# edenartlab/sd-lora-trainer

Measured on AMD Instinct MI355X. Metric: training images/sec, SDXL 1024px rank-16 LoRA, 1/2/4/8 GPU (job-parallel), higher is better.
Workload: dtype bf16

## Files before the change

### sd-lora-trainer_amd/csrc/attn.hip

```cpp
#include <cstdlib>
#include "common.h"
#include "../../include/sdlt_kernels.h"
#include "attn32.h"

namespace {

#ifdef SDLT_ATTN_TRACE
#define TR() do { if (tr) trb[trn++] = clock64(); } while (0)
#else
#define TR() do {} while (0)
#endif

constexpr float LOG2E = 1.4426950408889634f;

__device__ __forceinline__ bf16x8 pack8(const float* a, const float* b) {
  union { uint4 u; bf16x8 v; } c;
  c.u.x = pack2bf(a[0], a[1]); c.u.y = pack2bf(a[2], a[3]);
  c.u.z = pack2bf(b[0], b[1]); c.u.w = pack2bf(b[2], b[3]);
  return c.v;
}
__device__ __forceinline__ bf16x8 ld_frag_global(const bf16_t* p, bool ok) {
  union { uint4 u; bf16x8 v; } c;
  c.u = ok ? *(const uint4*)p : make_uint4(0, 0, 0, 0);
  return c.v;
// ... 1033 lines not shown
    return s;
  }();
  return sw;
}

struct AttnPlan {
  int route = 0;
  int dp = 64, ks = 1;
  bool dv48 = false, five = false, prep = false, splitsum = false;
  dim3 grid, grid2;
  int block = 256, smem = 0, smem2 = 0;
  int nq_roles = 0;
};
int attn32_ks(int env, bool two) { return env >= 4 ? 4 : env >= 2 ? 2 : env > 0 ? 1 : two ? 2 : 1; }

int attn_plan_fwd(const sdlt_attn_params& p, const AttnSwitches& sw, AttnPlan& pl) {
  int rc = attn_check(p, "sdlt_attn_fwd");
  if (rc) return rc;
  if (p.ldo % 4) SDLT_FAIL(SDLT_ERR_ALIGN, "sdlt_attn_fwd: ldo %% 4");
  pl = AttnPlan{};
  pl.dp = attn_dp(p.d);
  pl.grid = dim3((p.Nq + 63) / 64, p.H, p.B);
  if (sw.r32 && sdlt_attn32_ok(p) && ((uintptr_t)p.O % 16) == 0 && (p.ldo % 8) == 0) {
    pl.route = SDLT_ATTN_ROUTE_FWD32;
    pl.ks = attn32_ks(sw.ks32_fwd, p.Nk >= 128);
    pl.block = 128 * pl.ks;
    pl.smem = sdlt_attn32_fwd(pl.ks).smem;
    return SDLT_OK;
  }
  const bool ks2 = pl.dp == 64 && sw.ks == 2 && p.Nk >= 256 && (int64_t)pl.grid.x * pl.grid.y * pl.grid.z <= 512;
  pl.route = ks2 ? SDLT_ATTN_ROUTE_FWD16_KS2 : SDLT_ATTN_ROUTE_FWD16;
  pl.ks = ks2 ? 2 : 1;
  pl.dv48 = !ks2 && sw.dv48 && pl.dp == 64 && p.d <= 48;
  pl.block = 256 * pl.ks;
  pl.smem = smem_fwd(pl.dp, pl.ks);
  return SDLT_OK;
}

int attn_plan_bwd(const sdlt_attn_params& p, const AttnSwitches& sw, AttnPlan& pl) {
  int rc = attn_check_bwd(p, "sdlt_attn_bwd", false);
  if (rc) return rc;
  if (p.qsplit < 1) SDLT_FAIL(SDLT_ERR_SHAPE, "sdlt_attn_bwd: qsplit=%d", p.qsplit);
  if (!p.dK || !p.dV || (p.lddk % 4) || (p.lddv % 4) || (p.qsplit > 1 && (!p.dK32 || !p.dV32 || (p.ld32 % 4))))
    SDLT_FAIL(SDLT_ERR_SHAPE, "sdlt_attn_bwd: dK/dV outputs for qsplit=%d", p.qsplit);
  pl = AttnPlan{};
  pl.dp = attn_dp(p.d);
  const int tq = (p.Nq + 63) / 64, tk = (p.Nk + 63) / 64;
  if (p.qsplit > 1 && !p.causal && p.Nk <= 128 && p.Nkp <= 128 && pl.dp <= 96) {
    const bool roles = sw.roles && pl.dp == 64;
    pl.route = roles ? SDLT_ATTN_ROUTE_BWD_CROSS_ROLES : SDLT_ATTN_ROUTE_BWD_CROSS;
    pl.five = sw.five && p.Nk > 64 && p.Nk <= 80;
    if (roles) pl.nq_roles = p.qsplit / sw.qdiv > 0 ? p.qsplit / sw.qdiv : 1;
    pl.grid = dim3(pl.nq_roles + p.qsplit, p.H, p.B);
    pl.smem = roles ? smem_cross_roles(pl.dp) : smem_cross(pl.dp);
    pl.splitsum = !p.defer_splitsum;
    return SDLT_OK;
  }
  if (p.qsplit == 1 && !p.accumulate_dq && !p.accumulate_dk && (int64_t)(tq + tk) * p.H * p.B <= 2048) {
    const int64_t groups = (int64_t)p.B * p.Nqp * p.H;
    if (groups >= (1 << 22)) SDLT_FAIL(SDLT_ERR_UNSUPPORTED, "sdlt_attn_bwd: B * Nq * H = %lld rows (the D pre-pass indexes < 2^22)", (long long)groups);
    pl.prep = !p.d_ready;
    pl.grid = dim3(tq + tk, p.H, p.B);
    if (sw.r32 && sdlt_attn32_ok(p) && ((uintptr_t)p.L % 16) == 0 && ((uintptr_t)p.D % 16) == 0 &&
        (((uintptr_t)p.dQ | (uintptr_t)p.dK | (uintptr_t)p.dV) % 16) == 0 && ((p.lddq | p.lddk | p.lddv) % 8) == 0) {
      pl.route = SDLT_ATTN_ROUTE_BWD_BOTH32;
      pl.ks = attn32_ks(sw.ks32_bwd, p.Nk >= 128 && p.Nq >= 128);
      pl.block = 128 * pl.ks;
      pl.smem = sdlt_attn32_bwd_both(pl.ks).smem;
    } else {
      pl.route = SDLT_ATTN_ROUTE_BWD_BOTH16;
      pl.smem = smem_both(pl.dp);
    }
    return SDLT_OK;
  }
  if (p.accumulate_dq || p.accumulate_dk) SDLT_FAIL(SDLT_ERR_UNSUPPORTED, "sdlt_attn_bwd: accumulate_dq/dk exist for the single-pass cross-attention kernel only");
  if (p.qsplit > 1 && (((uintptr_t)p.dK32 | (uintptr_t)p.dV32) & 15 || (p.ld32 & 3) || ((p.H * p.d) & 3)))
    SDLT_FAIL(SDLT_ERR_ALIGN, "sdlt_attn_bwd: the dK / dV slabs of a query-split backward need 16-byte rows (ld32 %% 4, C %% 4)");
  pl.route = SDLT_ATTN_ROUTE_BWD_SPLIT;
  pl.dv48 = sw.dv48 && pl.dp == 64 && p.d <= 48;
  pl.grid = dim3(tq, p.H, p.B);
  pl.grid2 = dim3(tk * p.qsplit, p.H, p.B);
  pl.smem = smem_fwd(pl.dp);
  pl.smem2 = smem_both(pl.dp);
  pl.splitsum = p.qsplit > 1;
  return SDLT_OK;
}

// ... 135 lines not shown
```

### sd-lora-trainer_amd/csrc/attn32.h

```cpp
#pragma once
#include <hip/hip_runtime.h>
#include "../../include/sdlt_kernels.h"
bool sdlt_attn32_ok(const sdlt_attn_params& p);
struct sdlt_attn32_kernel { void (*fn)(const sdlt_attn_params); int smem; };
sdlt_attn32_kernel sdlt_attn32_fwd(int ks);
sdlt_attn32_kernel sdlt_attn32_bwd_both(int ks);
```

### sd-lora-trainer_amd/csrc/attn32.hip

```cpp
#include "common.h"
#include "../../include/sdlt_kernels.h"
#include "attn32.h"

namespace {

constexpr float LOG2E = 1.4426950408889634f;
typedef float f32x16 __attribute__((ext_vector_type(16)));
constexpr int TILE = 64 * 128;

__device__ __forceinline__ int sw32(int row) { return (((row >> 1) & 1) << 2) | ((row >> 2) & 3); }
__device__ __forceinline__ int rmap(int rho) { return (rho & 0x13) | ((rho & 4) << 1) | ((rho & 8) >> 1); }

struct WgId { int x, y, z; };
__device__ __forceinline__ WgId xcd_wg() {
  const int gx = gridDim.x, gy = gridDim.y, n = gx * gy * gridDim.z;
  const int L = blockIdx.x + gx * (blockIdx.y + gy * blockIdx.z);
  const int k = L & 7, slot = L >> 3, q = n >> 3, r = n & 7;
  const int logical = (k < r ? k * (q + 1) : r * (q + 1) + (k - r) * q) + slot;
  WgId w;
  const int t = div_small_u(logical, gx);
  w.x = logical - t * gx;
  w.z = gridDim.z == 1 ? 0 : div_small_u(t, gy);
  w.y = t - w.z * gy;
  return w;
}

__device__ __forceinline__ void tile_dma(const bf16_t* src, int64_t ld, char* dst, int w2, int lane) {
#pragma unroll
  for (int pc = 0; pc < 4; ++pc) {
    const int piece = w2 * 4 + pc;
    const int r = piece * 8 + (lane >> 3);
    glds16(src + (int64_t)r * ld + (((lane & 7) ^ sw32(r)) << 3), dst + piece * 1024);
  }
}

template <int OFF>
__device__ __forceinline__ bf16x8 lds_b128(uint32_t a) {
  bf16x8 v;
  asm volatile("ds_read_b128 %0, %1 offset:%2" : "=v"(v) : "v"(a), "n"(OFF));
  return v;
}
template <int OFF>
__device__ __forceinline__ bf16x4 lds_tr(uint32_t a) {
  bf16x4 v;
  asm volatile("ds_read_b64_tr_b16 %0, %1 offset:%2" : "=v"(v) : "v"(a), "n"(OFF));
  return v;
}
template <int N>
__device__ __forceinline__ void wait_lgkm() { asm volatile("s_waitcnt lgkmcnt(%0)" ::"n"(N) : "memory"); }
__device__ __forceinline__ void pin(bf16x8& v) { asm volatile("" : "+v"(v)); }
__device__ __forceinline__ void pin(bf16x4& v) { asm volatile("" : "+v"(v)); }
template <int BLK>
__device__ __forceinline__ void rows_issue(bf16x8 (&f)[4], uint32_t tile, const int (&row)[4]) {
#pragma unroll
  for (int kk = 0; kk < 4; ++kk) f[kk] = lds_b128<BLK * 4096>(tile + row[kk]);
}
__device__ __forceinline__ void rows_pin(bf16x8 (&f)[4]) {
#pragma unroll
  for (int kk = 0; kk < 4; ++kk) pin(f[kk]);
}
struct TrFrag { bf16x4 v[4]; };
template <int CH>
__device__ __forceinline__ void tr_issue(TrFrag& f, uint32_t tile, const int (&t1)[2], const int (&t2)[2]) {
  f.v[0] = lds_tr<CH * 2048>(tile + t1[0]);
  f.v[1] = lds_tr<CH * 2048>(tile + t2[0]);
  f.v[2] = lds_tr<CH * 2048>(tile + t1[1]);
  f.v[3] = lds_tr<CH * 2048>(tile + t2[1]);
}
__device__ __forceinline__ void tr_pin(TrFrag& f) {
#pragma unroll
  for (int k = 0; k < 4; ++k) pin(f.v[k]);
}
__device__ __forceinline__ bf16x8 tr_get(const TrFrag& f, int db) { return __builtin_shufflevector(f.v[2 * db], f.v[2 * db + 1], 0, 1, 2, 3, 4, 5, 6, 7); }
__device__ __forceinline__ uint32_t lds_addr(const char* p) { return (uint32_t)(uintptr_t)(__attribute__((address_space(3))) const char*)p; }
__device__ __forceinline__ bf16x8 ld8(const bf16_t* p) {
  union { uint4 u; bf16x8 v; } c;
  c.u = *(const uint4*)p;
  return c.v;
}
__device__ __forceinline__ bf16x8 pack8v(const f32x16& v, int c2) {
  union { uint4 u; bf16x8 b; } c;
  c.u.x = pack2bf(v[8 * c2 + 0], v[8 * c2 + 1]); c.u.y = pack2bf(v[8 * c2 + 2], v[8 * c2 + 3]);
  c.u.z = pack2bf(v[8 * c2 + 4], v[8 * c2 + 5]); c.u.w = pack2bf(v[8 * c2 + 6], v[8 * c2 + 7]);
  return c.b;
}
__device__ __forceinline__ float half_max(float v) {
  auto r = __builtin_amdgcn_permlane32_swap(__float_as_uint(v), __float_as_uint(v), false, false);
  return fmaxf(__uint_as_float(r[0]), __uint_as_float(r[1]));
}
__device__ __forceinline__ float half_sum(float v) {
  auto r = __builtin_amdgcn_permlane32_swap(__float_as_uint(v), __float_as_uint(v), false, false);
  return __uint_as_float(r[0]) + __uint_as_float(r[1]);
}
#ifndef SDLT_A32_STORE16
#define SDLT_A32_STORE16 1
#endif
__device__ __forceinline__ void store_pair(bf16_t* p, int hl, uint2 ev, uint2 od) {
#if SDLT_A32_STORE16
  auto x = __builtin_amdgcn_permlane32_swap(ev.x, od.x, false, false);
  auto y = __builtin_amdgcn_permlane32_swap(ev.y, od.y, false, false);
  *(uint4*)p = make_uint4(x[0], y[0], x[1], y[1]);
#else
  *(uint2*)(p - 4 * hl) = ev;
  *(uint2*)(p - 4 * hl + 8) = od;
#endif
}

__device__ __forceinline__ void wait_dma_barrier() {
  asm volatile("s_waitcnt vmcnt(0)" ::: "memory");
  __syncthreads();
}

struct FragOff {
  int row[4];
  int t1[2], t2[2];
};
__device__ __forceinline__ FragOff frag_offsets(int lane) {
  FragOff f;
  const int hl = lane >> 5, c = lane & 31, rr = rmap(c);
#pragma unroll
  for (int kk = 0; kk < 4; ++kk) f.row[kk] = rr * 128 + (((2 * kk + hl) ^ sw32(rr)) << 4);
  const int g = lane >> 4, i = lane & 15;
  const int R = 8 * (g >> 1) + (i >> 2), swl = (((i >> 3) & 1) << 2) | ((g >> 1) << 1), chl = 2 * (g & 1) + ((i & 3) >> 1);
#pragma unroll
  for (int db = 0; db < 2; ++db) {
    f.t1[db] = R * 128 + (((4 * db + chl) ^ swl) << 4) + (i & 1) * 8;
    f.t2[db] = (R + 4) * 128 + (((4 * db + chl) ^ swl ^ 1) << 4) + (i & 1) * 8;
  }
  return f;
}

#define MFMA32(a, b, c) __builtin_amdgcn_mfma_f32_32x32x16_bf16(a, b, c, 0, 0, 0)

#ifndef SDLT_A32_DMA_SPLIT
#define SDLT_A32_DMA_SPLIT 1
#endif

#ifdef SDLT_ATTN32_TRACE
#define TR32_DECL(BUF_, ON_) long long* tr_ = (long long*)(BUF_); int tn_ = 0; const bool tron_ = (ON_) && tr_ != nullptr
#define TR32() do { if (tron_ && tn_ < 500) { __builtin_amdgcn_sched_barrier(0); tr_[tn_++] = clock64(); __builtin_amdgcn_sched_barrier(0); } } while (0)
#else
#define TR32_DECL(BUF_, ON_)
#define TR32() do { } while (0)
#endif

template <int KS>
__global__ __launch_bounds__(128 * KS) void attn32_fwd_kernel(const sdlt_attn_params p) {
  extern __shared__ __attribute__((aligned(16))) char smem[];
  const WgId wg = xcd_wg();
  const int b = wg.z, h = wg.y, q0 = wg.x * 64;
  const int lane = threadIdx.x & 63, wv = __builtin_amdgcn_readfirstlane(threadIdx.x >> 6);
  const int grp = wv >> 1, w2 = wv & 1, hl = lane >> 5, c = lane & 31;
  const int hc = h * 64;
  const int q = q0 + w2 * 32 + c;
  const bf16_t* Kb = (const bf16_t*)p.K + (int64_t)b * p.Nkp * p.ldk + hc;
  const bf16_t* Vb = (const bf16_t*)p.V + (int64_t)b * p.Nkp * p.ldv + hc;
  char* ring = smem + grp * (4 * TILE);
  const int ntile = p.Nk >> 6, niter = (ntile + KS - 1) / KS;
  if (grp < ntile) {
    tile_dma(Kb + (int64_t)grp * 64 * p.ldk, p.ldk, ring, w2, lane);
    tile_dma(Vb + (int64_t)grp * 64 * p.ldv, p.ldv, ring + TILE, w2, lane);
  }
  bf16x8 qf[4];
  {
    const bf16_t* qp = (const bf16_t*)p.Q + ((int64_t)b * p.Nqp + q) * p.ldq + hc + 8 * hl;
#pragma unroll
    for (int kk = 0; kk < 4; ++kk) qf[kk] = ld8(qp + 16 * kk);
  }
  const FragOff fo = frag_offsets(lane);
  float m = -1e30f, lsum = 0.f;
  f32x16 o[2];
#pragma unroll
  for (int db = 0; db < 2; ++db)
#pragma unroll
    for (int r = 0; r < 16; ++r) o[db][r] = 0.f;
  const float sl2 = p.scale * LOG2E;
  TR32_DECL(p.D, wg.x == 0 && wg.y == 0 && wg.z == 0 && threadIdx.x == 0);
  TR32();
  wait_dma_barrier();
  for (int it = 0; it < niter; ++it) {
    TR32();
    const int t = it * KS + grp;
    const char* Ks = ring + (it & 1) * (2 * TILE);
    const char* Vs = Ks + TILE;
    char* nb = ring + ((it + 1) & 1) * (2 * TILE);
    const bool more = t + KS < ntile;
#if SDLT_A32_DMA_SPLIT == 0
    if (more) {
      tile_dma(Kb + (int64_t)(t + KS) * 64 * p.ldk, p.ldk, nb, w2, lane);
      tile_dma(Vb + (int64_t)(t + KS) * 64 * p.ldv, p.ldv, nb + TILE, w2, lane);
    }
#endif
    TR32();
    if (t < ntile) {
      const uint32_t ka = lds_addr(Ks), va = lds_addr(Vs);
      bf16x8 k0f[4], k1f[4];
      TrFrag vt[4];
      rows_issue<0>(k0f, ka, fo.row);
      rows_issue<1>(k1f, ka, fo.row);
      tr_issue<0>(vt[0], va, fo.t1, fo.t2);
      tr_issue<1>(vt[1], va, fo.t1, fo.t2);
      f32x16 s[2];
#pragma unroll
      for (int blk = 0; blk < 2; ++blk)
#pragma unroll
        for (int r = 0; r < 16; ++r) s[blk][r] = 0.f;
      wait_lgkm<12>();
      rows_pin(k0f);
#pragma unroll
      for (int kk = 0; kk < 4; ++kk) s[0] = MFMA32(k0f[kk], qf[kk], s[0]);
#if SDLT_A32_DMA_SPLIT
      if (more) tile_dma(Kb + (int64_t)(t + KS) * 64 * p.ldk, p.ldk, nb, w2, lane);
#endif
      tr_issue<2>(vt[2], va, fo.t1, fo.t2);
      tr_issue<3>(vt[3], va, fo.t1, fo.t2);
      wait_lgkm<15>();
      rows_pin(k1f);
#pragma unroll
      for (int kk = 0; kk < 4; ++kk) s[1] = MFMA32(k1f[kk], qf[kk], s[1]);
#if SDLT_A32_DMA_SPLIT
      if (more) tile_dma(Vb + (int64_t)(t + KS) * 64 * p.ldv, p.ldv, nb + TILE, w2, lane);
#endif
      __builtin_amdgcn_sched_barrier(0);
      TR32();
      float tmax = s[0][0];
#pragma unroll
      for (int blk = 0; blk < 2; ++blk)
#pragma unroll
        for (int r = 0; r < 16; ++r) tmax = fmaxf(tmax, s[blk][r]);
      tmax = half_max(tmax);
      const float mn = fmaxf(m, tmax * sl2);
      const float alpha = __builtin_amdgcn_exp2f(m - mn);
      m = mn;
      float rs = 0.f;
#pragma unroll
      for (int blk = 0; blk < 2; ++blk)
#pragma unroll
        for (int r = 0; r < 16; ++r) {
          const float pv = __builtin_amdgcn_exp2f(__builtin_fmaf(s[blk][r], sl2, -mn));
          s[blk][r] = pv;
          rs += pv;
        }
      lsum = lsum * alpha + rs;
#pragma unroll
      for (int db = 0; db < 2; ++db)
#pragma unroll
        for (int r = 0; r < 16; ++r) o[db][r] *= alpha;
      __builtin_amdgcn_sched_barrier(0);
      TR32();
      wait_lgkm<0>();
#pragma unroll
      for (int ch = 0; ch < 4; ++ch) tr_pin(vt[ch]);
#pragma unroll
      for (int ch = 0; ch < 4; ++ch) {
        const bf16x8 pf = pack8v(s[ch >> 1], ch & 1);
#pragma unroll
        for (int db = 0; db < 2; ++db) o[db] = MFMA32(tr_get(vt[ch], db), pf, o[db]);
      }
    }
    TR32();
    wait_dma_barrier();
  }
  TR32();
  lsum = half_sum(lsum);
  if constexpr (KS > 1) {
    float* mg = (float*)smem + (((grp - 1) * 2 + w2) * 64 + lane) * 36;
    if (grp > 0) {
      mg[0] = m;
      mg[1] = lsum;
#pragma unroll
      for (int db = 0; db < 2; ++db)
#pragma unroll
        for (int j = 0; j < 4; ++j) *(f32x4*)(mg + 4 + db * 16 + j * 4) = (f32x4){o[db][4 * j], o[db][4 * j + 1], o[db][4 * j + 2], o[db][4 * j + 3]};
    }
    __syncthreads();
    if (grp > 0) return;
#pragma unroll
    for (int g2 = 1; g2 < KS; ++g2) {
      const float* sg = (const float*)smem + (((g2 - 1) * 2 + w2) * 64 + lane) * 36;
      const float m1 = sg[0], l1 = sg[1];
      const float mn = fmaxf(m, m1), a0 = __builtin_amdgcn_exp2f(m - mn), a1 = __builtin_amdgcn_exp2f(m1 - mn);
      m = mn;
      lsum = lsum * a0 + l1 * a1;
#pragma unroll
// ... 14 lines not shown
  bf16_t* op = (bf16_t*)p.O + ((int64_t)b * p.Nqp + q) * p.ldo + hc + 8 * hl;
#pragma unroll
  for (int db = 0; db < 2; ++db)
#pragma unroll
    for (int jp = 0; jp < 2; ++jp) {
      uint2 w[2];
#pragma unroll
      for (int e = 0; e < 2; ++e) {
        const int j = 2 * jp + e;
        w[e].x = pack2bf(o[db][4 * j] * inv, o[db][4 * j + 1] * inv);
        w[e].y = pack2bf(o[db][4 * j + 2] * inv, o[db][4 * j + 3] * inv);
      }
      store_pair(op + 32 * db + 16 * jp, hl, w[0], w[1]);
    }
}

template <int KS>
__device__ __forceinline__ void attn32_dq_body(const sdlt_attn_params& p, char* smem, const int bx, const WgId wg) {
  const int b = wg.z, h = wg.y, q0 = bx * 64;
  const int lane = threadIdx.x & 63, wv = __builtin_amdgcn_readfirstlane(threadIdx.x >> 6);
  const int grp = wv >> 1, w2 = wv & 1, hl = lane >> 5, c = lane & 31;
  const int hc = h * 64;
  const int q = q0 + w2 * 32 + c;
  const bf16_t* Kb = (const bf16_t*)p.K + (int64_t)b * p.Nkp * p.ldk + hc;
  const bf16_t* Vb = (const bf16_t*)p.V + (int64_t)b * p.Nkp * p.ldv + hc;
  char* ring = smem + grp * (4 * TILE);
  const int ntile = p.Nk >> 6, niter = (ntile + KS - 1) / KS;
  if (grp < ntile) {
    tile_dma(Kb + (int64_t)grp * 64 * p.ldk, p.ldk, ring, w2, lane);
    tile_dma(Vb + (int64_t)grp * 64 * p.ldv, p.ldv, ring + TILE, w2, lane);
  }
  bf16x8 qf[4], gf[4];
  {
    const bf16_t* qp = (const bf16_t*)p.Q + ((int64_t)b * p.Nqp + q) * p.ldq + hc + 8 * hl;
    const bf16_t* gp = (const bf16_t*)p.dO + ((int64_t)b * p.Nqp + q) * p.lddo + hc + 8 * hl;
#pragma unroll
    for (int kk = 0; kk < 4; ++kk) {
      qf[kk] = ld8(qp + 16 * kk);
      gf[kk] = ld8(gp + 16 * kk);
    }
  }
  const float Lq = p.L[((int64_t)b * p.H + h) * p.Nq + q] * LOG2E;
  const float Dq = p.D[((int64_t)b * p.H + h) * p.Nq + q];
  const FragOff fo = frag_offsets(lane);
  f32x16 dq[2];
#pragma unroll
  for (int db = 0; db < 2; ++db)
#pragma unroll
    for (int r = 0; r < 16; ++r) dq[db][r] = 0.f;
  const float sl2 = p.scale * LOG2E;
  TR32_DECL(p.dK32, bx == 0 && wg.y == 0 && wg.z == 0 && threadIdx.x == 0);
  TR32();
  wait_dma_barrier();
  for (int it = 0; it < niter; ++it) {
    TR32();
    const int t = it * KS + grp;
    const char* Ks = ring + (it & 1) * (2 * TILE);
    const char* Vs = Ks + TILE;
    char* nb = ring + ((it + 1) & 1) * (2 * TILE);
    const bool more = t + KS < ntile;
#if SDLT_A32_DMA_SPLIT == 0
    if (more) {
      tile_dma(Kb + (int64_t)(t + KS) * 64 * p.ldk, p.ldk, nb, w2, lane);
      tile_dma(Vb + (int64_t)(t + KS) * 64 * p.ldv, p.ldv, nb + TILE, w2, lane);
    }
#endif
    TR32();
    if (t < ntile) {
      const uint32_t ka = lds_addr(Ks), va = lds_addr(Vs);
      bf16x8 kr[2][4], vr[2][4];
      TrFrag kt[2][2];
      rows_issue<0>(kr[0], ka, fo.row);
      rows_issue<0>(vr[0], va, fo.row);
      tr_issue<0>(kt[0][0], ka, fo.t1, fo.t2);
      tr_issue<1>(kt[0][1], ka, fo.t1, fo.t2);
#pragma unroll
      for (int blk = 0; blk < 2; ++blk) {
        f32x16 s, dp;
#pragma unroll
        for (int r = 0; r < 16; ++r) { s[r] = 0.f; dp[r] = 0.f; }
        wait_lgkm<8>();
        rows_pin(kr[blk]);
        rows_pin(vr[blk]);
#pragma unroll
        for (int kk = 0; kk < 4; ++kk) {
          s = MFMA32(kr[blk][kk], qf[kk], s);
          dp = MFMA32(vr[blk][kk], gf[kk], dp);
        }
        if (blk == 0) {
          rows_issue<1>(kr[1], ka, fo.row);
          rows_issue<1>(vr[1], va, fo.row);
        }
#if SDLT_A32_DMA_SPLIT
        if (more) {
          if (blk == 0) tile_dma(Kb + (int64_t)(t + KS) * 64 * p.ldk, p.ldk, nb, w2, lane);
          else tile_dma(Vb + (int64_t)(t + KS) * 64 * p.ldv, p.ldv, nb + TILE, w2, lane);
        }
#endif
        __builtin_amdgcn_sched_barrier(0);
        TR32();
#pragma unroll
        for (int r = 0; r < 16; ++r) {
          const float pv = __builtin_amdgcn_exp2f(__builtin_fmaf(s[r], sl2, -Lq));
          s[r] = pv * (dp[r] - Dq);
        }
        __builtin_amdgcn_sched_barrier(0);
        TR32();
        if (blk == 0) wait_lgkm<8>(); else wait_lgkm<0>();
        tr_pin(kt[blk][0]);
        tr_pin(kt[blk][1]);
#pragma unroll
        for (int c2 = 0; c2 < 2; ++c2) {
          const bf16x8 dsf = pack8v(s, c2);
#pragma unroll
          for (int db = 0; db < 2; ++db) dq[db] = MFMA32(tr_get(kt[blk][c2], db), dsf, dq[db]);
        }
        if (blk == 0) {
          tr_issue<2>(kt[1][0], ka, fo.t1, fo.t2);
          tr_issue<3>(kt[1][1], ka, fo.t1, fo.t2);
        }
        TR32();
      }
    }
    wait_dma_barrier();
  }
  TR32();
  if constexpr (KS > 1) {
    float* mg = (float*)smem + (((grp - 1) * 2 + w2) * 64 + lane) * 36;
    if (grp > 0) {
#pragma unroll
      for (int db = 0; db < 2; ++db)
#pragma unroll
        for (int j = 0; j < 4; ++j) *(f32x4*)(mg + db * 16 + j * 4) = (f32x4){dq[db][4 * j], dq[db][4 * j + 1], dq[db][4 * j + 2], dq[db][4 * j + 3]};
    }
    __syncthreads();
    if (grp > 0) return;
#pragma unroll
    for (int g2 = 1; g2 < KS; ++g2) {
      const float* sg = (const float*)smem + (((g2 - 1) * 2 + w2) * 64 + lane) * 36;
#pragma unroll
      for (int db = 0; db < 2; ++db)
#pragma unroll
        for (int j = 0; j < 4; ++j) {
          const f32x4 o1 = *(const f32x4*)(sg + db * 16 + j * 4);
#pragma unroll
          for (int r = 0; r < 4; ++r) dq[db][4 * j + r] += o1[r];
        }
// ... 3 lines not shown
#pragma unroll
  for (int db = 0; db < 2; ++db)
#pragma unroll
    for (int jp = 0; jp < 2; ++jp) {
      uint2 w[2];
#pragma unroll
      for (int e = 0; e < 2; ++e) {
        const int j = 2 * jp + e;
        w[e].x = pack2bf(dq[db][4 * j] * p.scale, dq[db][4 * j + 1] * p.scale);
        w[e].y = pack2bf(dq[db][4 * j + 2] * p.scale, dq[db][4 * j + 3] * p.scale);
      }
      store_pair(op + 32 * db + 16 * jp, hl, w[0], w[1]);
    }
}

template <int KS>
__device__ __forceinline__ void attn32_dkdv_body(const sdlt_attn_params& p, char* smem, const int bx, const WgId wg) {
  constexpr int RING = 2 * (2 * TILE + 512);
  const int b = wg.z, h = wg.y, k0 = bx * 64;
  const int lane = threadIdx.x & 63, wv = __builtin_amdgcn_readfirstlane(threadIdx.x >> 6);
  const int grp = wv >> 1, w2 = wv & 1, hl = lane >> 5, c = lane & 31;
  const int hc = h * 64;
  const int key = k0 + w2 * 32 + c;
  const bf16_t* Qb = (const bf16_t*)p.Q + (int64_t)b * p.Nqp * p.ldq + hc;
  const bf16_t* Gb = (const bf16_t*)p.dO + (int64_t)b * p.Nqp * p.lddo + hc;
  const float* Lb = p.L + ((int64_t)b * p.H + h) * p.Nq;
  const float* Db = p.D + ((int64_t)b * p.H + h) * p.Nq;
  char* ring = smem + grp * RING;
  const int ntile = p.Nq >> 6, niter = (ntile + KS - 1) / KS;
  auto stage_q = [&](int t, char* buf) { tile_dma(Qb + (int64_t)t * 64 * p.ldq, p.ldq, buf, w2, lane); };
  auto stage_g = [&](int t, char* buf) {
    tile_dma(Gb + (int64_t)t * 64 * p.lddo, p.lddo, buf + TILE, w2, lane);
    if (lane < 16) glds16((w2 ? Db : Lb) + t * 64 + lane * 4, buf + 2 * TILE + w2 * 256);
  };
  auto stage = [&](int t, char* buf) { stage_q(t, buf); stage_g(t, buf); };
  if (grp < ntile) stage(grp, ring);
  bf16x8 kf[4], vf[4];
  {
    const bf16_t* kp = (const bf16_t*)p.K + ((int64_t)b * p.Nkp + key) * p.ldk + hc + 8 * hl;
    const bf16_t* vp = (const bf16_t*)p.V + ((int64_t)b * p.Nkp + key) * p.ldv + hc + 8 * hl;
#pragma unroll
    for (int kk = 0; kk < 4; ++kk) {
      kf[kk] = ld8(kp + 16 * kk);
      vf[kk] = ld8(vp + 16 * kk);
    }
  }
  const FragOff fo = frag_offsets(lane);
  f32x16 dk[2], dv[2];
#pragma unroll
  for (int db = 0; db < 2; ++db)
#pragma unroll
    for (int r = 0; r < 16; ++r) { dk[db][r] = 0.f; dv[db][r] = 0.f; }
  const float sl2 = p.scale * LOG2E;
  TR32_DECL(p.dK32 ? p.dK32 + 1024 : nullptr, bx == 0 && wg.y == 0 && wg.z == 0 && threadIdx.x == 0);
  TR32();
  wait_dma_barrier();
  for (int it = 0; it < niter; ++it) {
    TR32();
    const int t = it * KS + grp;
    const char* Qs = ring + (it & 1) * (2 * TILE + 512);
    const char* Gs = Qs + TILE;
    const float* Ls = (const float*)(Gs + TILE);
    const float* Ds = Ls + 64;
    char* nb = ring + ((it + 1) & 1) * (2 * TILE + 512);
    const bool more = t + KS < ntile;
#if SDLT_A32_DMA_SPLIT == 0
    if (more) stage(t + KS, nb);
#endif
    TR32();
    if (t < ntile) {
      const uint32_t qa = lds_addr(Qs), ga = lds_addr(Gs);
      bf16x8 qr[2][4], gr[2][4];
      TrFrag gt[2][2], qt[2][2];
      rows_issue<0>(qr[0], qa, fo.row);
      rows_issue<0>(gr[0], ga, fo.row);
      tr_issue<0>(gt[0][0], ga, fo.t1, fo.t2);
      tr_issue<0>(qt[0][0], qa, fo.t1, fo.t2);
#pragma unroll
      for (int blk = 0; blk < 2; ++blk) {
        f32x16 s, dp;
#pragma unroll
        for (int r = 0; r < 16; ++r) { s[r] = 0.f; dp[r] = 0.f; }
        wait_lgkm<8>();
        rows_pin(qr[blk]);
        rows_pin(gr[blk]);
#pragma unroll
        for (int kk = 0; kk < 4; ++kk) {
          s = MFMA32(qr[blk][kk], kf[kk], s);
          dp = MFMA32(gr[blk][kk], vf[kk], dp);
        }
        if (blk == 0) {
          tr_issue<1>(gt[0][1], ga, fo.t1, fo.t2);
          tr_issue<1>(qt[0][1], qa, fo.t1, fo.t2);
        } else {
          tr_issue<3>(gt[1][1], ga, fo.t1, fo.t2);
          tr_issue<3>(qt[1][1], qa, fo.t1, fo.t2);
        }
#if SDLT_A32_DMA_SPLIT
        if (more) {
          if (blk == 0) stage_q(t + KS, nb);
          else stage_g(t + KS, nb);
        }
#endif
        __builtin_amdgcn_sched_barrier(0);
        TR32();
#pragma unroll
        for (int c2 = 0; c2 < 2; ++c2) {
          const int qb = blk * 32 + c2 * 16 + 8 * hl;
          const f32x4 l0 = *(const f32x4*)(Ls + qb), l1 = *(const f32x4*)(Ls + qb + 4);
          const f32x4 d0 = *(const f32x4*)(Ds + qb), d1 = *(const f32x4*)(Ds + qb + 4);
#pragma unroll
          for (int e = 0; e < 8; ++e) {
            const float lq = (e < 4 ? l0[e & 3] : l1[e & 3]) * LOG2E, dd = e < 4 ? d0[e & 3] : d1[e & 3];
            const float pv = __builtin_amdgcn_exp2f(__builtin_fmaf(s[8 * c2 + e], sl2, -lq));
            s[8 * c2 + e] = pv;
            dp[8 * c2 + e] = pv * (dp[8 * c2 + e] - dd);
          }
        }
        __builtin_amdgcn_sched_barrier(0);
        TR32();
        wait_lgkm<8>();
        tr_pin(gt[blk][0]);
        tr_pin(qt[blk][0]);
        {
          const bf16x8 pf = pack8v(s, 0), dsf = pack8v(dp, 0);
#pragma unroll
          for (int db = 0; db < 2; ++db) {
            dv[db] = MFMA32(tr_get(gt[blk][0], db), pf, dv[db]);
            dk[db] = MFMA32(tr_get(qt[blk][0], db), dsf, dk[db]);
          }
        }
        if (blk == 0) {
          rows_issue<1>(qr[1], qa, fo.row);
          rows_issue<1>(gr[1], ga, fo.row);
          tr_issue<2>(gt[1][0], ga, fo.t1, fo.t2);
          tr_issue<2>(qt[1][0], qa, fo.t1, fo.t2);
          wait_lgkm<15>();
        } else {
          wait_lgkm<0>();
        }
        tr_pin(gt[blk][1]);
        tr_pin(qt[blk][1]);
        {
          const bf16x8 pf = pack8v(s, 1), dsf = pack8v(dp, 1);
#pragma unroll
          for (int db = 0; db < 2; ++db) {
            dv[db] = MFMA32(tr_get(gt[blk][1], db), pf, dv[db]);
            dk[db] = MFMA32(tr_get(qt[blk][1], db), dsf, dk[db]);
          }
        }
        TR32();
      }
    }
    wait_dma_barrier();
  }
  TR32();
  if constexpr (KS > 1) {
    float* mg = (float*)smem + (((grp - 1) * 2 + w2) * 64 + lane) * 68;
    if (grp > 0) {
#pragma unroll
      for (int db = 0; db < 2; ++db)
#pragma unroll
        for (int j = 0; j < 4; ++j) {
          *(f32x4*)(mg + db * 16 + j * 4) = (f32x4){dk[db][4 * j], dk[db][4 * j + 1], dk[db][4 * j + 2], dk[db][4 * j + 3]};
          *(f32x4*)(mg + 32 + db * 16 + j * 4) = (f32x4){dv[db][4 * j], dv[db][4 * j + 1], dv[db][4 * j + 2], dv[db][4 * j + 3]};
        }
    }
    __syncthreads();
    if (grp > 0) return;
#pragma unroll
    for (int g2 = 1; g2 < KS; ++g2) {
      const float* sg = (const float*)smem + (((g2 - 1) * 2 + w2) * 64 + lane) * 68;
#pragma unroll
      for (int db = 0; db < 2; ++db)
#pragma unroll
        for (int j = 0; j < 4; ++j) {
          const f32x4 a = *(const f32x4*)(sg + db * 16 + j * 4), e = *(const f32x4*)(sg + 32 + db * 16 + j * 4);
// ... 21 lines not shown
        wv[e].x = pack2bf(dv[db][4 * j], dv[db][4 * j + 1]);
        wv[e].y = pack2bf(dv[db][4 * j + 2], dv[db][4 * j + 3]);
      }
      store_pair(kp2 + 32 * db + 16 * jp, hl, wk[0], wk[1]);
      store_pair(vp2 + 32 * db + 16 * jp, hl, wv[0], wv[1]);
    }
}

template <int KS>
__global__ __launch_bounds__(128 * KS) void attn32_bwd_both_kernel(const sdlt_attn_params p) {
  extern __shared__ __attribute__((aligned(16))) char smem[];
  const int ndq = p.Nq >> 6;
  const WgId wg = xcd_wg();
  if (wg.x < ndq) attn32_dq_body<KS>(p, smem, wg.x, wg);
  else attn32_dkdv_body<KS>(p, smem, wg.x - ndq, wg);
}

}

bool sdlt_attn32_ok(const sdlt_attn_params& p) {
  return p.d == 64 && !p.causal && p.Nq >= 64 && p.Nk >= 64 && (p.Nq % 64) == 0 && (p.Nk % 64) == 0 && p.Nqp >= p.Nq && p.Nkp >= p.Nk;
}

sdlt_attn32_kernel sdlt_attn32_fwd(int ks) {
  static void (*const fn[3])(const sdlt_attn_params) = {attn32_fwd_kernel<4>, attn32_fwd_kernel<2>, attn32_fwd_kernel<1>};
  return {fn[ks == 4 ? 0 : ks == 2 ? 1 : 2], ks * 4 * TILE};
}

sdlt_attn32_kernel sdlt_attn32_bwd_both(int ks) {
  static void (*const fn[3])(const sdlt_attn_params) = {attn32_bwd_both_kernel<4>, attn32_bwd_both_kernel<2>, attn32_bwd_both_kernel<1>};
  return {fn[ks == 4 ? 0 : ks == 2 ? 1 : 2], ks * 2 * (2 * TILE + 512)};
}
```

Before: 24.13.

## Use buffer-resource LDS loads and unroll ring stages for constant LDS offsets

Global-to-LDS tile copies in the attn32 forward and backward kernels now go through per-head buffer resource descriptors with precomputed 32-bit per-lane offsets. The per-tile address arithmetic reduces to a scalar offset, replacing 64-bit pointer math on every issue. The main loop is unrolled by two so each double-buffer stage has compile-time LDS offsets folded into the ds_read immediates, which saves VGPRs and ALU work. In exchange, a host check now rejects heads whose rows span 4 GiB or more, and the code size grows.

```diff
diff --git a/sd-lora-trainer_amd/csrc/attn.hip b/sd-lora-trainer_amd/csrc/attn.hip
--- a/sd-lora-trainer_amd/csrc/attn.hip
+++ b/sd-lora-trainer_amd/csrc/attn.hip
@@ -1079,6 +1079,7 @@
   pl.dp = attn_dp(p.d);
   pl.grid = dim3((p.Nq + 63) / 64, p.H, p.B);
   if (sw.r32 && sdlt_attn32_ok(p) && ((uintptr_t)p.O % 16) == 0 && (p.ldo % 8) == 0) {
+    if (!sdlt_attn32_span_ok(p, false)) SDLT_FAIL(SDLT_ERR_UNSUPPORTED, "sdlt_attn_fwd: the K / V rows of one head span >= 4 GiB (Nk=%d ldk=%lld ldv=%lld)", p.Nk, (long long)p.ldk, (long long)p.ldv);
     pl.route = SDLT_ATTN_ROUTE_FWD32;
     pl.ks = attn32_ks(sw.ks32_fwd, p.Nk >= 128);
     pl.block = 128 * pl.ks;
@@ -1120,6 +1121,9 @@
     pl.grid = dim3(tq + tk, p.H, p.B);
     if (sw.r32 && sdlt_attn32_ok(p) && ((uintptr_t)p.L % 16) == 0 && ((uintptr_t)p.D % 16) == 0 &&
         (((uintptr_t)p.dQ | (uintptr_t)p.dK | (uintptr_t)p.dV) % 16) == 0 && ((p.lddq | p.lddk | p.lddv) % 8) == 0) {
+      if (!sdlt_attn32_span_ok(p, true))
+        SDLT_FAIL(SDLT_ERR_UNSUPPORTED, "sdlt_attn_bwd: the Q / dO / K / V rows of one head span >= 4 GiB (Nq=%d Nk=%d ldq=%lld lddo=%lld ldk=%lld ldv=%lld)", p.Nq, p.Nk,
+                  (long long)p.ldq, (long long)p.lddo, (long long)p.ldk, (long long)p.ldv);
       pl.route = SDLT_ATTN_ROUTE_BWD_BOTH32;
       pl.ks = attn32_ks(sw.ks32_bwd, p.Nk >= 128 && p.Nq >= 128);
       pl.block = 128 * pl.ks;
diff --git a/sd-lora-trainer_amd/csrc/attn32.h b/sd-lora-trainer_amd/csrc/attn32.h
--- a/sd-lora-trainer_amd/csrc/attn32.h
+++ b/sd-lora-trainer_amd/csrc/attn32.h
@@ -2,6 +2,7 @@
 #include <hip/hip_runtime.h>
 #include "../../include/sdlt_kernels.h"
 bool sdlt_attn32_ok(const sdlt_attn_params& p);
+bool sdlt_attn32_span_ok(const sdlt_attn_params& p, bool bwd);
 struct sdlt_attn32_kernel { void (*fn)(const sdlt_attn_params); int smem; };
 sdlt_attn32_kernel sdlt_attn32_fwd(int ks);
 sdlt_attn32_kernel sdlt_attn32_bwd_both(int ks);
diff --git a/sd-lora-trainer_amd/csrc/attn32.hip b/sd-lora-trainer_amd/csrc/attn32.hip
--- a/sd-lora-trainer_amd/csrc/attn32.hip
+++ b/sd-lora-trainer_amd/csrc/attn32.hip
@@ -25,14 +25,28 @@
   return w;
 }
 
-__device__ __forceinline__ void tile_dma(const bf16_t* src, int64_t ld, char* dst, int w2, int lane) {
+typedef __amdgpu_buffer_rsrc_t rsrc_t;
+__device__ __forceinline__ rsrc_t head_rsrc(const void* base, uint32_t bytes) {
+  return __builtin_amdgcn_make_buffer_rsrc(const_cast<void*>(base), 0, bytes, 0x00020000);
+}
+typedef __attribute__((address_space(3))) void* lds_ptr;
+struct DmaOff { uint32_t v[4]; };
+__device__ __forceinline__ DmaOff dma_offsets(int64_t ld, int w2, int lane) {
+  DmaOff d;
 #pragma unroll
   for (int pc = 0; pc < 4; ++pc) {
-    const int piece = w2 * 4 + pc;
-    const int r = piece * 8 + (lane >> 3);
-    glds16(src + (int64_t)r * ld + (((lane & 7) ^ sw32(r)) << 3), dst + piece * 1024);
-  }
-}
+    const int r = (w2 * 4 + pc) * 8 + (lane >> 3);
+    d.v[pc] = (uint32_t)r * ((uint32_t)ld * 2u) + (uint32_t)((((lane & 7) ^ sw32(r)) << 4) - pc * 1024);
+  }
+  return d;
+}
+__device__ __forceinline__ void tile_dma(rsrc_t rs, const DmaOff& d, uint32_t soff, char* dst) {
+  __builtin_amdgcn_raw_ptr_buffer_load_lds(rs, (lds_ptr)dst, 16, d.v[0], soff, 0, 0);
+  __builtin_amdgcn_raw_ptr_buffer_load_lds(rs, (lds_ptr)dst, 16, d.v[1], soff, 1024, 0);
+  __builtin_amdgcn_raw_ptr_buffer_load_lds(rs, (lds_ptr)dst, 16, d.v[2], soff, 2048, 0);
+  __builtin_amdgcn_raw_ptr_buffer_load_lds(rs, (lds_ptr)dst, 16, d.v[3], soff, 3072, 0);
+}
+template <int V> struct IntC { static constexpr int value = V; };
 
 template <int OFF>
 __device__ __forceinline__ bf16x8 lds_b128(uint32_t a) {
@@ -50,22 +64,22 @@
 __device__ __forceinline__ void wait_lgkm() { asm volatile("s_waitcnt lgkmcnt(%0)" ::"n"(N) : "memory"); }
 __device__ __forceinline__ void pin(bf16x8& v) { asm volatile("" : "+v"(v)); }
 __device__ __forceinline__ void pin(bf16x4& v) { asm volatile("" : "+v"(v)); }
-template <int BLK>
-__device__ __forceinline__ void rows_issue(bf16x8 (&f)[4], uint32_t tile, const int (&row)[4]) {
-#pragma unroll
-  for (int kk = 0; kk < 4; ++kk) f[kk] = lds_b128<BLK * 4096>(tile + row[kk]);
+template <int TOFF, int BLK>
+__device__ __forceinline__ void rows_issue(bf16x8 (&f)[4], const uint32_t (&row)[4]) {
+#pragma unroll
+  for (int kk = 0; kk < 4; ++kk) f[kk] = lds_b128<TOFF + BLK * 4096>(row[kk]);
 }
 __device__ __forceinline__ void rows_pin(bf16x8 (&f)[4]) {
 #pragma unroll
   for (int kk = 0; kk < 4; ++kk) pin(f[kk]);
 }
 struct TrFrag { bf16x4 v[4]; };
-template <int CH>
-__device__ __forceinline__ void tr_issue(TrFrag& f, uint32_t tile, const int (&t1)[2], const int (&t2)[2]) {
-  f.v[0] = lds_tr<CH * 2048>(tile + t1[0]);
-  f.v[1] = lds_tr<CH * 2048>(tile + t2[0]);
-  f.v[2] = lds_tr<CH * 2048>(tile + t1[1]);
-  f.v[3] = lds_tr<CH * 2048>(tile + t2[1]);
+template <int TOFF, int CH>
+__device__ __forceinline__ void tr_issue(TrFrag& f, const uint32_t (&t1)[2], const uint32_t (&t2)[2]) {
+  f.v[0] = lds_tr<TOFF + CH * 2048>(t1[0]);
+  f.v[1] = lds_tr<TOFF + CH * 2048>(t2[0]);
+  f.v[2] = lds_tr<TOFF + CH * 2048>(t1[1]);
+  f.v[3] = lds_tr<TOFF + CH * 2048>(t2[1]);
 }
 __device__ __forceinline__ void tr_pin(TrFrag& f) {
 #pragma unroll
@@ -112,20 +126,20 @@
 }
 
 struct FragOff {
-  int row[4];
-  int t1[2], t2[2];
+  uint32_t row[4];
+  uint32_t t1[2], t2[2];
 };
-__device__ __forceinline__ FragOff frag_offsets(int lane) {
+__device__ __forceinline__ FragOff frag_offsets(int lane, uint32_t base) {
   FragOff f;
   const int hl = lane >> 5, c = lane & 31, rr = rmap(c);
 #pragma unroll
-  for (int kk = 0; kk < 4; ++kk) f.row[kk] = rr * 128 + (((2 * kk + hl) ^ sw32(rr)) << 4);
+  for (int kk = 0; kk < 4; ++kk) f.row[kk] = base + rr * 128 + (((2 * kk + hl) ^ sw32(rr)) << 4);
   const int g = lane >> 4, i = lane & 15;
   const int R = 8 * (g >> 1) + (i >> 2), swl = (((i >> 3) & 1) << 2) | ((g >> 1) << 1), chl = 2 * (g & 1) + ((i & 3) >> 1);
 #pragma unroll
   for (int db = 0; db < 2; ++db) {
-    f.t1[db] = R * 128 + (((4 * db + chl) ^ swl) << 4) + (i & 1) * 8;
-    f.t2[db] = (R + 4) * 128 + (((4 * db + chl) ^ swl ^ 1) << 4) + (i & 1) * 8;
+    f.t1[db] = base + R * 128 + (((4 * db + chl) ^ swl) << 4) + (i & 1) * 8;
+    f.t2[db] = base + (R + 4) * 128 + (((4 * db + chl) ^ swl ^ 1) << 4) + (i & 1) * 8;
   }
   return f;
 }
@@ -153,13 +167,16 @@
   const int grp = wv >> 1, w2 = wv & 1, hl = lane >> 5, c = lane & 31;
   const int hc = h * 64;
   const int q = q0 + w2 * 32 + c;
-  const bf16_t* Kb = (const bf16_t*)p.K + (int64_t)b * p.Nkp * p.ldk + hc;
-  const bf16_t* Vb = (const bf16_t*)p.V + (int64_t)b * p.Nkp * p.ldv + hc;
+  const int ntile = p.Nk >> 6, niter = (ntile + KS - 1) / KS;
+  const rsrc_t Kr = head_rsrc((const bf16_t*)p.K + (int64_t)b * p.Nkp * p.ldk + hc, (uint32_t)((int64_t)(p.Nk - 1) * p.ldk * 2 + 128));
+  const rsrc_t Vr = head_rsrc((const bf16_t*)p.V + (int64_t)b * p.Nkp * p.ldv + hc, (uint32_t)((int64_t)(p.Nk - 1) * p.ldv * 2 + 128));
+  const DmaOff kd = dma_offsets(p.ldk, w2, lane), vd = dma_offsets(p.ldv, w2, lane);
+  const uint32_t kstep = (uint32_t)p.ldk * 128u, vstep = (uint32_t)p.ldv * 128u;
   char* ring = smem + grp * (4 * TILE);
-  const int ntile = p.Nk >> 6, niter = (ntile + KS - 1) / KS;
+  char* wdst = ring + w2 * 4096;
   if (grp < ntile) {
-    tile_dma(Kb + (int64_t)grp * 64 * p.ldk, p.ldk, ring, w2, lane);
-    tile_dma(Vb + (int64_t)grp * 64 * p.ldv, p.ldv, ring + TILE, w2, lane);
+    tile_dma(Kr, kd, grp * kstep, wdst);
+    tile_dma(Vr, vd, grp * vstep, wdst + TILE);
   }
   bf16x8 qf[4];
   {
@@ -167,7 +184,7 @@
 #pragma unroll
     for (int kk = 0; kk < 4; ++kk) qf[kk] = ld8(qp + 16 * kk);
   }
-  const FragOff fo = frag_offsets(lane);
+  const FragOff fo = frag_offsets(lane, lds_addr(ring));
   float m = -1e30f, lsum = 0.f;
   f32x16 o[2];
 #pragma unroll
@@ -178,28 +195,25 @@
   TR32_DECL(p.D, wg.x == 0 && wg.y == 0 && wg.z == 0 && threadIdx.x == 0);
   TR32();
   wait_dma_barrier();
-  for (int it = 0; it < niter; ++it) {
+  auto stage = [&](auto stc, const int it) {
+    constexpr int ST = decltype(stc)::value, KO = ST * (2 * TILE), VO = KO + TILE, NB = (1 - ST) * (2 * TILE);
     TR32();
     const int t = it * KS + grp;
-    const char* Ks = ring + (it & 1) * (2 * TILE);
-    const char* Vs = Ks + TILE;
-    char* nb = ring + ((it + 1) & 1) * (2 * TILE);
     const bool more = t + KS < ntile;
 #if SDLT_A32_DMA_SPLIT == 0
     if (more) {
-      tile_dma(Kb + (int64_t)(t + KS) * 64 * p.ldk, p.ldk, nb, w2, lane);
-      tile_dma(Vb + (int64_t)(t + KS) * 64 * p.ldv, p.ldv, nb + TILE, w2, lane);
+      tile_dma(Kr, kd, (t + KS) * kstep, wdst + NB);
+      tile_dma(Vr, vd, (t + KS) * vstep, wdst + NB + TILE);
     }
 #endif
     TR32();
     if (t < ntile) {
-      const uint32_t ka = lds_addr(Ks), va = lds_addr(Vs);
       bf16x8 k0f[4], k1f[4];
       TrFrag vt[4];
-      rows_issue<0>(k0f, ka, fo.row);
-      rows_issue<1>(k1f, ka, fo.row);
-      tr_issue<0>(vt[0], va, fo.t1, fo.t2);
-      tr_issue<1>(vt[1], va, fo.t1, fo.t2);
+      rows_issue<KO, 0>(k0f, fo.row);
+      rows_issue<KO, 1>(k1f, fo.row);
+      tr_issue<VO, 0>(vt[0], fo.t1, fo.t2);
+      tr_issue<VO, 1>(vt[1], fo.t1, fo.t2);
       f32x16 s[2];
 #pragma unroll
       for (int blk = 0; blk < 2; ++blk)
@@ -210,16 +224,16 @@
 #pragma unroll
       for (int kk = 0; kk < 4; ++kk) s[0] = MFMA32(k0f[kk], qf[kk], s[0]);
 #if SDLT_A32_DMA_SPLIT
-      if (more) tile_dma(Kb + (int64_t)(t + KS) * 64 * p.ldk, p.ldk, nb, w2, lane);
-#endif
-      tr_issue<2>(vt[2], va, fo.t1, fo.t2);
-      tr_issue<3>(vt[3], va, fo.t1, fo.t2);
+      if (more) tile_dma(Kr, kd, (t + KS) * kstep, wdst + NB);
+#endif
+      tr_issue<VO, 2>(vt[2], fo.t1, fo.t2);
+      tr_issue<VO, 3>(vt[3], fo.t1, fo.t2);
       wait_lgkm<15>();
       rows_pin(k1f);
 #pragma unroll
       for (int kk = 0; kk < 4; ++kk) s[1] = MFMA32(k1f[kk], qf[kk], s[1]);
 #if SDLT_A32_DMA_SPLIT
-      if (more) tile_dma(Vb + (int64_t)(t + KS) * 64 * p.ldv, p.ldv, nb + TILE, w2, lane);
+      if (more) tile_dma(Vr, vd, (t + KS) * vstep, wdst + NB + TILE);
 #endif
       __builtin_amdgcn_sched_barrier(0);
       TR32();
@@ -260,6 +274,11 @@
     }
     TR32();
     wait_dma_barrier();
+  };
+  for (int it = 0; it < niter; it += 2) {
+    stage(IntC<0>{}, it);
+    if (it + 1 >= niter) break;
+    stage(IntC<1>{}, it + 1);
   }
   TR32();
   lsum = half_sum(lsum);
@@ -320,13 +339,16 @@
   const int grp = wv >> 1, w2 = wv & 1, hl = lane >> 5, c = lane & 31;
   const int hc = h * 64;
   const int q = q0 + w2 * 32 + c;
-  const bf16_t* Kb = (const bf16_t*)p.K + (int64_t)b * p.Nkp * p.ldk + hc;
-  const bf16_t* Vb = (const bf16_t*)p.V + (int64_t)b * p.Nkp * p.ldv + hc;
+  const int ntile = p.Nk >> 6, niter = (ntile + KS - 1) / KS;
+  const rsrc_t Kr = head_rsrc((const bf16_t*)p.K + (int64_t)b * p.Nkp * p.ldk + hc, (uint32_t)((int64_t)(p.Nk - 1) * p.ldk * 2 + 128));
+  const rsrc_t Vr = head_rsrc((const bf16_t*)p.V + (int64_t)b * p.Nkp * p.ldv + hc, (uint32_t)((int64_t)(p.Nk - 1) * p.ldv * 2 + 128));
+  const DmaOff kd = dma_offsets(p.ldk, w2, lane), vd = dma_offsets(p.ldv, w2, lane);
+  const uint32_t kstep = (uint32_t)p.ldk * 128u, vstep = (uint32_t)p.ldv * 128u;
   char* ring = smem + grp * (4 * TILE);
-  const int ntile = p.Nk >> 6, niter = (ntile + KS - 1) / KS;
+  char* wdst = ring + w2 * 4096;
   if (grp < ntile) {
-    tile_dma(Kb + (int64_t)grp * 64 * p.ldk, p.ldk, ring, w2, lane);
-    tile_dma(Vb + (int64_t)grp * 64 * p.ldv, p.ldv, ring + TILE, w2, lane);
+    tile_dma(Kr, kd, grp * kstep, wdst);
+    tile_dma(Vr, vd, grp * vstep, wdst + TILE);
   }
   bf16x8 qf[4], gf[4];
   {
@@ -340,7 +362,7 @@
   }
   const float Lq = p.L[((int64_t)b * p.H + h) * p.Nq + q] * LOG2E;
   const float Dq = p.D[((int64_t)b * p.H + h) * p.Nq + q];
-  const FragOff fo = frag_offsets(lane);
+  const FragOff fo = frag_offsets(lane, lds_addr(ring));
   f32x16 dq[2];
 #pragma unroll
   for (int db = 0; db < 2; ++db)
@@ -350,28 +372,25 @@
   TR32_DECL(p.dK32, bx == 0 && wg.y == 0 && wg.z == 0 && threadIdx.x == 0);
   TR32();
   wait_dma_barrier();
-  for (int it = 0; it < niter; ++it) {
+  auto stage = [&](auto stc, const int it) {
+    constexpr int ST = decltype(stc)::value, KO = ST * (2 * TILE), VO = KO + TILE, NB = (1 - ST) * (2 * TILE);
     TR32();
     const int t = it * KS + grp;
-    const char* Ks = ring + (it & 1) * (2 * TILE);
-    const char* Vs = Ks + TILE;
-    char* nb = ring + ((it + 1) & 1) * (2 * TILE);
     const bool more = t + KS < ntile;
 #if SDLT_A32_DMA_SPLIT == 0
     if (more) {
-      tile_dma(Kb + (int64_t)(t + KS) * 64 * p.ldk, p.ldk, nb, w2, lane);
-      tile_dma(Vb + (int64_t)(t + KS) * 64 * p.ldv, p.ldv, nb + TILE, w2, lane);
+      tile_dma(Kr, kd, (t + KS) * kstep, wdst + NB);
+      tile_dma(Vr, vd, (t + KS) * vstep, wdst + NB + TILE);
     }
 #endif
     TR32();
     if (t < ntile) {
-      const uint32_t ka = lds_addr(Ks), va = lds_addr(Vs);
       bf16x8 kr[2][4], vr[2][4];
       TrFrag kt[2][2];
-      rows_issue<0>(kr[0], ka, fo.row);
-      rows_issue<0>(vr[0], va, fo.row);
-      tr_issue<0>(kt[0][0], ka, fo.t1, fo.t2);
-      tr_issue<1>(kt[0][1], ka, fo.t1, fo.t2);
+      rows_issue<KO, 0>(kr[0], fo.row);
+      rows_issue<VO, 0>(vr[0], fo.row);
+      tr_issue<KO, 0>(kt[0][0], fo.t1, fo.t2);
+      tr_issue<KO, 1>(kt[0][1], fo.t1, fo.t2);
 #pragma unroll
       for (int blk = 0; blk < 2; ++blk) {
         f32x16 s, dp;
@@ -386,13 +405,13 @@
           dp = MFMA32(vr[blk][kk], gf[kk], dp);
         }
         if (blk == 0) {
-          rows_issue<1>(kr[1], ka, fo.row);
-          rows_issue<1>(vr[1], va, fo.row);
+          rows_issue<KO, 1>(kr[1], fo.row);
+          rows_issue<VO, 1>(vr[1], fo.row);
         }
 #if SDLT_A32_DMA_SPLIT
         if (more) {
-          if (blk == 0) tile_dma(Kb + (int64_t)(t + KS) * 64 * p.ldk, p.ldk, nb, w2, lane);
-          else tile_dma(Vb + (int64_t)(t + KS) * 64 * p.ldv, p.ldv, nb + TILE, w2, lane);
+          if (blk == 0) tile_dma(Kr, kd, (t + KS) * kstep, wdst + NB);
+          else tile_dma(Vr, vd, (t + KS) * vstep, wdst + NB + TILE);
         }
 #endif
         __builtin_amdgcn_sched_barrier(0);
@@ -414,13 +433,18 @@
           for (int db = 0; db < 2; ++db) dq[db] = MFMA32(tr_get(kt[blk][c2], db), dsf, dq[db]);
         }
         if (blk == 0) {
-          tr_issue<2>(kt[1][0], ka, fo.t1, fo.t2);
-          tr_issue<3>(kt[1][1], ka, fo.t1, fo.t2);
+          tr_issue<KO, 2>(kt[1][0], fo.t1, fo.t2);
+          tr_issue<KO, 3>(kt[1][1], fo.t1, fo.t2);
         }
         TR32();
       }
     }
     wait_dma_barrier();
+  };
+  for (int it = 0; it < niter; it += 2) {
+    stage(IntC<0>{}, it);
+    if (it + 1 >= niter) break;
+    stage(IntC<1>{}, it + 1);
   }
   TR32();
   if constexpr (KS > 1) {
@@ -470,19 +494,24 @@
   const int grp = wv >> 1, w2 = wv & 1, hl = lane >> 5, c = lane & 31;
   const int hc = h * 64;
   const int key = k0 + w2 * 32 + c;
-  const bf16_t* Qb = (const bf16_t*)p.Q + (int64_t)b * p.Nqp * p.ldq + hc;
-  const bf16_t* Gb = (const bf16_t*)p.dO + (int64_t)b * p.Nqp * p.lddo + hc;
-  const float* Lb = p.L + ((int64_t)b * p.H + h) * p.Nq;
-  const float* Db = p.D + ((int64_t)b * p.H + h) * p.Nq;
+  const int ntile = p.Nq >> 6, niter = (ntile + KS - 1) / KS;
+  const rsrc_t Qr = head_rsrc((const bf16_t*)p.Q + (int64_t)b * p.Nqp * p.ldq + hc, (uint32_t)((int64_t)(p.Nq - 1) * p.ldq * 2 + 128));
+  const rsrc_t Gr = head_rsrc((const bf16_t*)p.dO + (int64_t)b * p.Nqp * p.lddo + hc, (uint32_t)((int64_t)(p.Nq - 1) * p.lddo * 2 + 128));
+  const rsrc_t Sr = head_rsrc((w2 ? p.D : p.L) + ((int64_t)b * p.H + h) * p.Nq, (uint32_t)p.Nq * 4u);
+  const DmaOff qd = dma_offsets(p.ldq, w2, lane), gd = dma_offsets(p.lddo, w2, lane);
+  const uint32_t qstep = (uint32_t)p.ldq * 128u, gstep = (uint32_t)p.lddo * 128u;
   char* ring = smem + grp * RING;
-  const int ntile = p.Nq >> 6, niter = (ntile + KS - 1) / KS;
-  auto stage_q = [&](int t, char* buf) { tile_dma(Qb + (int64_t)t * 64 * p.ldq, p.ldq, buf, w2, lane); };
-  auto stage_g = [&](int t, char* buf) {
-    tile_dma(Gb + (int64_t)t * 64 * p.lddo, p.lddo, buf + TILE, w2, lane);
-    if (lane < 16) glds16((w2 ? Db : Lb) + t * 64 + lane * 4, buf + 2 * TILE + w2 * 256);
+  char* wdst = ring + w2 * 4096;
+  char* sdst = ring + 2 * TILE + w2 * 256;
+  auto stage_q = [&](int t, char* buf) { tile_dma(Qr, qd, t * qstep, buf); };
+  auto stage_g = [&](int t, char* buf, char* sbuf) {
+    tile_dma(Gr, gd, t * gstep, buf + TILE);
+    if (lane < 16) __builtin_amdgcn_raw_ptr_buffer_load_lds(Sr, (lds_ptr)sbuf, 16, lane * 16, t * 256, 0, 0);
   };
-  auto stage = [&](int t, char* buf) { stage_q(t, buf); stage_g(t, buf); };
-  if (grp < ntile) stage(grp, ring);
+  if (grp < ntile) {
+    stage_q(grp, wdst);
+    stage_g(grp, wdst, sdst);
+  }
   bf16x8 kf[4], vf[4];
   {
     const bf16_t* kp = (const bf16_t*)p.K + ((int64_t)b * p.Nkp + key) * p.ldk + hc + 8 * hl;
@@ -493,7 +522,7 @@
       vf[kk] = ld8(vp + 16 * kk);
     }
   }
-  const FragOff fo = frag_offsets(lane);
+  const FragOff fo = frag_offsets(lane, lds_addr(ring));
   f32x16 dk[2], dv[2];
 #pragma unroll
   for (int db = 0; db < 2; ++db)
@@ -503,27 +532,27 @@
   TR32_DECL(p.dK32 ? p.dK32 + 1024 : nullptr, bx == 0 && wg.y == 0 && wg.z == 0 && threadIdx.x == 0);
   TR32();
   wait_dma_barrier();
-  for (int it = 0; it < niter; ++it) {
+  auto stage = [&](auto stc, const int it) {
+    constexpr int ST = decltype(stc)::value, QO = ST * (2 * TILE + 512), GO = QO + TILE, NB = (1 - ST) * (2 * TILE + 512);
     TR32();
     const int t = it * KS + grp;
-    const char* Qs = ring + (it & 1) * (2 * TILE + 512);
-    const char* Gs = Qs + TILE;
-    const float* Ls = (const float*)(Gs + TILE);
+    const float* Ls = (const float*)(ring + GO + TILE);
     const float* Ds = Ls + 64;
-    char* nb = ring + ((it + 1) & 1) * (2 * TILE + 512);
     const bool more = t + KS < ntile;
 #if SDLT_A32_DMA_SPLIT == 0
-    if (more) stage(t + KS, nb);
+    if (more) {
+      stage_q(t + KS, wdst + NB);
+      stage_g(t + KS, wdst + NB, sdst + NB);
+    }
 #endif
     TR32();
     if (t < ntile) {
-      const uint32_t qa = lds_addr(Qs), ga = lds_addr(Gs);
       bf16x8 qr[2][4], gr[2][4];
       TrFrag gt[2][2], qt[2][2];
-      rows_issue<0>(qr[0], qa, fo.row);
-      rows_issue<0>(gr[0], ga, fo.row);
-      tr_issue<0>(gt[0][0], ga, fo.t1, fo.t2);
-      tr_issue<0>(qt[0][0], qa, fo.t1, fo.t2);
+      rows_issue<QO, 0>(qr[0], fo.row);
+      rows_issue<GO, 0>(gr[0], fo.row);
+      tr_issue<GO, 0>(gt[0][0], fo.t1, fo.t2);
+      tr_issue<QO, 0>(qt[0][0], fo.t1, fo.t2);
 #pragma unroll
       for (int blk = 0; blk < 2; ++blk) {
         f32x16 s, dp;
@@ -538,16 +567,16 @@
           dp = MFMA32(gr[blk][kk], vf[kk], dp);
         }
         if (blk == 0) {
-          tr_issue<1>(gt[0][1], ga, fo.t1, fo.t2);
-          tr_issue<1>(qt[0][1], qa, fo.t1, fo.t2);
+          tr_issue<GO, 1>(gt[0][1], fo.t1, fo.t2);
+          tr_issue<QO, 1>(qt[0][1], fo.t1, fo.t2);
         } else {
-          tr_issue<3>(gt[1][1], ga, fo.t1, fo.t2);
-          tr_issue<3>(qt[1][1], qa, fo.t1, fo.t2);
+          tr_issue<GO, 3>(gt[1][1], fo.t1, fo.t2);
+          tr_issue<QO, 3>(qt[1][1], fo.t1, fo.t2);
         }
 #if SDLT_A32_DMA_SPLIT
         if (more) {
-          if (blk == 0) stage_q(t + KS, nb);
-          else stage_g(t + KS, nb);
+          if (blk == 0) stage_q(t + KS, wdst + NB);
+          else stage_g(t + KS, wdst + NB, sdst + NB);
         }
 #endif
         __builtin_amdgcn_sched_barrier(0);
@@ -579,10 +608,10 @@
           }
         }
         if (blk == 0) {
-          rows_issue<1>(qr[1], qa, fo.row);
-          rows_issue<1>(gr[1], ga, fo.row);
-          tr_issue<2>(gt[1][0], ga, fo.t1, fo.t2);
-          tr_issue<2>(qt[1][0], qa, fo.t1, fo.t2);
+          rows_issue<QO, 1>(qr[1], fo.row);
+          rows_issue<GO, 1>(gr[1], fo.row);
+          tr_issue<GO, 2>(gt[1][0], fo.t1, fo.t2);
+          tr_issue<QO, 2>(qt[1][0], fo.t1, fo.t2);
           wait_lgkm<15>();
         } else {
           wait_lgkm<0>();
@@ -601,6 +630,11 @@
       }
     }
     wait_dma_barrier();
+  };
+  for (int it = 0; it < niter; it += 2) {
+    stage(IntC<0>{}, it);
+    if (it + 1 >= niter) break;
+    stage(IntC<1>{}, it + 1);
   }
   TR32();
   if constexpr (KS > 1) {
@@ -668,6 +702,11 @@
   return p.d == 64 && !p.causal && p.Nq >= 64 && p.Nk >= 64 && (p.Nq % 64) == 0 && (p.Nk % 64) == 0 && p.Nqp >= p.Nq && p.Nkp >= p.Nk;
 }
 
+bool sdlt_attn32_span_ok(const sdlt_attn_params& p, bool bwd) {
+  auto fits = [](int64_t rows, int64_t ld) { return ld >= 64 && (rows - 1) * ld * 2 + 128 < ((int64_t)1 << 32); };
+  return fits(p.Nk, p.ldk) && fits(p.Nk, p.ldv) && (!bwd || (fits(p.Nq, p.ldq) && fits(p.Nq, p.lddo)));
+}
+
 sdlt_attn32_kernel sdlt_attn32_fwd(int ks) {
   static void (*const fn[3])(const sdlt_attn_params) = {attn32_fwd_kernel<4>, attn32_fwd_kernel<2>, attn32_fwd_kernel<1>};
   return {fn[ks == 4 ? 0 : ks == 2 ? 1 : 2], ks * 4 * TILE};
```

Result: no change. 24.30, median of 6 (+0.7%).
